# dusanerdeljan/stereo-depth

Measured on AMD Instinct MI355X. Metric: disparity maps/sec (stereo pairs/sec) at 1242x375 D=128, higher is better.
Workload: dtype f32

## Files before the change

stereo-depth_amd/build.py:

```python
from __future__ import annotations

import glob
import hashlib
import os
import shutil
import subprocess
import sys
from concurrent.futures import ThreadPoolExecutor

HERE = os.path.dirname(os.path.abspath(__file__))
CSRC = os.path.join(HERE, "csrc")
OBJ = os.path.join(CSRC, "build")
INCLUDE = os.path.join(os.path.dirname(HERE), "include")
LIB = os.path.join(HERE, "libstereo_mi355x.so")
FLAGS = ["--offload-arch=gfx950", "-O3", "-std=c++17", "-ffp-contract=off", "-fno-slp-vectorize", "-fPIC",
         "-Wall", "-Wno-pass-failed"]
PER_FILE_FLAGS = {"tu_capture.hip": ["-mllvm", "-pragma-unroll-threshold=65536"]}


def hipcc() -> str:
    for cand in (shutil.which("hipcc"), "/opt/rocm/bin/hipcc"):
        if cand and os.path.exists(cand):
            return cand
    raise RuntimeError("hipcc not found: cannot build libstereo_mi355x.so")


def sources():
    return sorted(glob.glob(os.path.join(CSRC, "*.hip")))


def _flags():
    extra = os.environ.get("SMX_EXTRA_FLAGS", "").split()
    return FLAGS + extra + ["-I", INCLUDE]


def _deps(depfile: str):
    try:
        txt = open(depfile).read().replace("\\\n", " ")
    except OSError:
        return None
    return [t for t in txt.split(":", 1)[1].split() if t]


def _stale(src: str, obj: str, stamp: str) -> bool:
    if not os.path.exists(obj):
        return True
    try:
        if open(obj + ".flags").read() != stamp:
            return True
    except OSError:
        return True
    deps = _deps(obj[:-2] + ".d")
    if deps is None:
        return True
    t = os.path.getmtime(obj)
    return any((not os.path.exists(d)) or os.path.getmtime(d) > t for d in deps + [src])


def build(force: bool = False, verbose: bool = False, variant: str = "") -> str:
    global LIB, OBJ
    if variant:
        LIB = os.path.join(HERE, f"libstereo_mi355x.{variant}.so")
        OBJ = os.path.join(CSRC, "build", variant)
    cc, flags = hipcc(), _flags()
    stamp = hashlib.sha256(" ".join([cc] + flags + [repr(sorted(PER_FILE_FLAGS.items()))]).encode()).hexdigest()
    try:
        fresh = (not force and open(LIB + ".flags").read() == stamp and
                 all(os.path.getmtime(f) <= os.path.getmtime(LIB)
                     for f in glob.glob(os.path.join(CSRC, "*.*")) + glob.glob(os.path.join(INCLUDE, "*.h")) + [__file__]))
    except OSError:
        fresh = False
    if fresh:
        return LIB
    os.makedirs(OBJ, exist_ok=True)
    jobs = []
    for src in sources():
        obj = os.path.join(OBJ, os.path.basename(src)[:-4] + ".o")
        if force or _stale(src, obj, stamp):
            jobs.append((src, obj))

    def compile_one(job):
        src, obj = job
        cmd = [cc] + flags + PER_FILE_FLAGS.get(os.path.basename(src), []) + ["-c", "-MD", "-MF", obj[:-2] + ".d", "-o", obj, src]
        if verbose:
            print(" ".join(cmd), flush=True)
        r = subprocess.run(cmd, capture_output=True, text=True)
        if r.returncode != 0:
            raise RuntimeError(f"hipcc failed on {os.path.basename(src)}:\n" + r.stdout + r.stderr)
        if r.stderr.strip() and verbose:
            print(r.stderr, file=sys.stderr)
        open(obj + ".flags", "w").write(stamp)

    if jobs:
        with ThreadPoolExecutor(max_workers=min(len(jobs), os.cpu_count() or 4, 8)) as pool:
            list(pool.map(compile_one, jobs))
    objs = [os.path.join(OBJ, os.path.basename(s)[:-4] + ".o") for s in sources()]
    if jobs or not os.path.exists(LIB) or any(os.path.getmtime(o) > os.path.getmtime(LIB) for o in objs):
        cmd = [cc, "--offload-arch=gfx950", "-shared", "-fPIC", "-o", LIB] + objs
        if verbose:
            print(" ".join(cmd), flush=True)
        r = subprocess.run(cmd, capture_output=True, text=True)
        if r.returncode != 0:
            raise RuntimeError("link failed:\n" + r.stdout + r.stderr)
    open(LIB + ".flags", "w").write(stamp)
    return LIB


if __name__ == "__main__":
    variant = next((a.split("=", 1)[1] for a in sys.argv if a.startswith("--variant=")), "")
    print(build(force="--force" in sys.argv, verbose="-v" in sys.argv or "--force" in sys.argv, variant=variant))
```

stereo-depth_amd/csrc/k_match_fast.h:

```cpp
#pragma once
#include "smx_common.h"

namespace smx {

constexpr int FA_HALO = 11;
constexpr int FA_VALID = 64 - 2 * FA_HALO;
#ifndef SMX_FA_WAVES
#define SMX_FA_WAVES 4
#endif
constexpr int FA_WAVES = SMX_FA_WAVES;
#ifndef SMX_FA_DS_WAVES
#define SMX_FA_DS_WAVES 8
#endif
constexpr int FA_DS_WAVES = SMX_FA_DS_WAVES;
#ifndef SMX_FA_TH
#define SMX_FA_TH 24
#endif
constexpr int FA_TH = SMX_FA_TH;
#ifndef SMX_FA_TH_SMALL
#define SMX_FA_TH_SMALL 8
#endif
constexpr int FA_TH_SMALL = SMX_FA_TH_SMALL;
constexpr int FA_TH_SMALL_TALL = 12;
constexpr int FA_TH_SMALL_MID = 10;
// ... 330 lines not shown
                            best[o] = __builtin_fmaxf(best[o], agg.x);
                            argb_update(o & 3, arg[o >> 2], agg.y, best[o], dvb);
                            best[o] = __builtin_fmaxf(best[o], agg.y);
                        } else {
                            const float m = __builtin_fmaxf(__builtin_fmaxf(best[o], agg.x), agg.y);
                            const int dsel = (agg.x == m) ? d : d + 1;
                            arg[o] = m > best[o] ? dsel : arg[o];
                            best[o] = m;
                        }
#endif
                    }
                }
            }
            s2 = s1;
            s1 = s0;
            k2 = k1;
            k1 = k0;
        }
        if ((rr_ % SMX_FA_SB_PERIOD) == SMX_FA_SB_PERIOD - 1)
            __builtin_amdgcn_sched_barrier(0);
    }
}

constexpr int FA_STAT_WG_STRIDE_DS = 16;
template <bool DSPLIT>
__device__ __forceinline__ void fast_stats_report(const MatchParams &p, int b, int wg_lin, int wv, int marches, bool window) {
    if (!p.fast_stats || b % p.fast_stride != 0) return;
    if (DSPLIT && wg_lin % FA_STAT_WG_STRIDE_DS != 0) return;
    const bool win = window && (!DSPLIT || wv == 0);
    const unsigned long long v = ((unsigned long long)(unsigned)marches << 24) | (win ? 1ull : 0ull);
    if (v != 0ull) (void)__hip_atomic_fetch_add(p.fast_stats, v, __ATOMIC_RELAXED, __HIP_MEMORY_SCOPE_AGENT);
}

template <int TH, int PR, bool P1ONLY, bool DSPLIT, int PK16, bool ARGB = false, bool DENSE = false>
__device__ __forceinline__ void match_fast_body(const MatchParams &p, const BlockIdx3 &blk) {
    static_assert(!DENSE || !P1ONLY, "the dense form is a pass 1 with neighbours: min_disparity = 0");
    static_assert(!DENSE || !DSPLIT || !ARGB, "latency shape: one register per winner");
    constexpr int NW = DSPLIT ? FA_DS_WAVES : FA_WAVES;
    constexpr int WGCOLS = DSPLIT ? 64 : FA_WGCOLS;
    constexpr int ND = PR - WGCOLS + 1;
    const int b = blk.z;

    extern __shared__ __attribute__((aligned(16))) unsigned short fsmem[];
    unsigned short *Lt = fsmem;
    unsigned short *Rt = fsmem + (TH + 22) * FA_PL;
    unsigned *bits = (unsigned *)(Rt + (TH + 22) * PR);
    const int BW = fast_bitwords(p.Dd);

    const int tid = threadIdx.x;
    const int lane = tid & 63;
    const int wv = tid >> 6;
    const int h = p.h, w = p.w, Dd = p.Dd;
    const int cwg0 = blk.x * (DSPLIT ? 1 : FA_WAVES) * FA_VALID;
    const int cw0 = cwg0 + (DSPLIT ? 0 : wv * FA_VALID);
    const int wcol = DSPLIT ? 0 : wv * FA_VALID;
    const bool active = cw0 < w;
    const int x0 = blk.y * TH;
    const int col = cw0 - FA_HALO + lane;
    const float *Lp = p.Ld + (size_t)b * h * w;
    const float *Rp = p.Rd + (size_t)b * h * w;
    const float unit = p.unit;

    FastLane ln;
    ln.xch = (float *)(bits + NW * BW) + wv * FA_XCH_FLOATS;
    ln.c255 = (unsigned)(255.0f * unit);
    ln.inv = 1.0f / (unit * unit * unit);
    ln.store_ok = active && lane >= FA_HALO && lane < FA_HALO + FA_VALID && col < w;
    ln.rows_ok = min(TH, h - x0);
    ln.plane = (size_t)p.B * h * w;
    ln.row0 = ((size_t)b * h + x0) * w;
    ln.colidx = ln.store_ok ? col : 0;
    ln.lptr = Lt + wcol + lane;

// ... 5 lines not shown
    float dfirst[DENSE && DSPLIT ? TH : 1];
#pragma unroll
    for (int o = 0; o < (DENSE ? TH : 1); ++o) { dmb[o] = 0.f; dma[o] = 0.f; dcp[o] = 0.f; }
#pragma unroll
    for (int o = 0; o < (DENSE && DSPLIT ? TH : 1); ++o) dfirst[o] = 0.f;

    fast_stage<(WGCOLS + 63) / 64, NW>(Lt, FA_PL, Lp, h, w, x0 - FA_HALO, cwg0 - FA_HALO, TH + 22, WGCOLS, unit, wv, lane);
    for (int e = tid; e < NW * BW; e += 64 * NW) bits[e] = 0u;

    auto stage_right = [&](int d0, int nd) {
        __syncthreads();
        const int cbase = cwg0 - FA_HALO - (p.dmin + d0 + nd - 1);
        fast_stage<(PR + 63) / 64, NW>(Rt, PR, Rp, h, w, x0 - FA_HALO, cbase, TH + 22, WGCOLS + nd - 1, unit, wv, lane);
        __syncthreads();
    };

    for (int d0 = 0; d0 < Dd; d0 += ND) {
        const int nd = min(ND, Dd - d0);
        stage_right(d0, nd);
        if (active) {
            const int q4 = ((nd + 2 * NW - 1) / (2 * NW)) * 2;
            const int dd_lo = DSPLIT ? min(nd, wv * q4) : 0;
            const int dd_hi = DSPLIT ? min(nd, dd_lo + q4) : nd;
            for (int dd = dd_lo; dd < dd_hi; dd += 2) {
                ln.rptr = Rt + wcol + lane + (nd - 1 - dd);
                if constexpr (DENSE)
                    fast_pass_pair<TH, PR, P1ONLY, PK16, 0, ARGB, true>(p, ln, d0 + dd, dd + 1 < dd_hi, best, arg, nullptr, 0, nullptr,
                                                                         0, 0, 0, 0, nullptr, nullptr, ~0u, dmb, dma, dcp,
                                                                         DSPLIT && dd == dd_lo ? dfirst : nullptr);
                else
                    fast_pass_pair<TH, PR, P1ONLY, PK16, 0, ARGB>(p, ln, d0 + dd, dd + 1 < dd_hi, best, arg);
            }
        }
    }
    if (ARGB) {
        int packed[(TH + 3) / 4];
#pragma unroll
        for (int o = 0; o < (TH + 3) / 4; ++o) packed[o] = arg[o];
#pragma unroll
        for (int o = 0; o < TH; ++o) arg[o] = (packed[o >> 2] >> (8 * (o & 3))) & 0xff;
    }
    float *mrg = (float *)(bits + NW * BW) + NW * FA_XCH_FLOATS;
    if constexpr (DSPLIT && DENSE) {
        constexpr int MR = fast_merge_rows(TH), R2 = (NW * MR * 2) / (NW * 6);
        static_assert(R2 >= 1 && R2 <= NW, "merge buffer: at least one row of six values per wave");
        const int q4 = ((Dd + 2 * NW - 1) / (2 * NW)) * 2;
        const int nk = (Dd + q4 - 1) / q4;
#pragma unroll 1
        for (int o0 = 0; o0 < TH; o0 += R2) {
            __syncthreads();
#pragma unroll
            for (int o = 0; o < TH; ++o) {
                if (o >= o0 && o < o0 + R2) {
                    float *q = mrg + ((size_t)(wv * R2 + (o - o0)) * 64 + lane) * 6;
                    q[0] = best[o]; q[1] = __int_as_float(arg[o]); q[2] = dmb[o]; q[3] = dma[o]; q[4] = dfirst[o]; q[5] = dcp[o];
                }
            }
            __syncthreads();
            const int j = wv;
            if (j < R2 && o0 + j < ln.rows_ok && ln.store_ok) {
                auto M = [&](int k, int f) { return mrg[((size_t)(k * R2 + j) * 64 + lane) * 6 + f]; };
                float bb = SMX_FLT_MIN;
                int aa = 0, kw = 0;
                for (int k = 0; k < nk; ++k) {
                    const float bk = M(k, 0);
                    const bool g = bk > bb;
// ... 174 lines not shown
#endif
    if (fl.form == FAST_DENSE_SMALL) {
        if constexpr (DSPLIT && TH == FA_TH_SMALL_TALL) launch_match_fast_k<TH, PR, false, true, false, true>(fl.pk, grid, block, lds, p, s);
    } else if (fl.form == FAST_DENSE) {
        if constexpr (!DSPLIT && ARGB && TH <= FA_DENSE_MAX_TH) launch_match_fast_k<TH, PR, false, false, ARGB, true>(fl.pk, grid, block, lds, p, s);
    } else if (fl.form == FAST_PASS1_ONLY) {
        launch_match_fast_k<TH, PR, true, DSPLIT, ARGB, false>(fl.pk, grid, block, lds, p, s);
    } else {
        launch_match_fast_k<TH, PR, false, DSPLIT, ARGB, false>(fl.pk, grid, block, lds, p, s);
    }
}

template <int TH, int PR, bool DSPLIT>
inline void launch_match_fast_t(const FastLaunch &fl, const MatchParams &p, int n, hipStream_t s) {
    if constexpr (DSPLIT) {
        launch_match_fast_a<TH, PR, true, false>(fl, p, n, s);
    } else if constexpr (PR == 256 || PR == FA_MID_PITCH) {
        launch_match_fast_a<TH, PR, false, true>(fl, p, n, s);
    } else {
        if (fl.argb) launch_match_fast_a<TH, PR, false, true>(fl, p, n, s);
        else launch_match_fast_a<TH, PR, false, false>(fl, p, n, s);
    }
}

__host__ __device__ constexpr int fast_tall_pitch(int Dd) { return Dd <= FA_WIDE_FROM ? 256 : (Dd <= FA_MID_UPTO ? FA_MID_PITCH : 320); }

template <int TH>
inline void launch_match_fast_tall(const FastLaunch &fl, const MatchParams &p, int n, hipStream_t s) {
    if (fl.pitch == 256) launch_match_fast_t<TH, 256, false>(fl, p, n, s);
    else if (fl.pitch == FA_MID_PITCH) launch_match_fast_t<TH, FA_MID_PITCH, false>(fl, p, n, s);
    else launch_match_fast_t<TH, 320, false>(fl, p, n, s);
}

struct FastPlan {
    bool small;
    int th;
    bool wide;
};

inline FastPlan match_fast_plan(const MatchParams &p, int n, int cus) {
    FastPlan pl{};
    const long wgs_tall = (long)((p.w + FA_VALID * FA_WAVES - 1) / (FA_VALID * FA_WAVES)) * ((p.h + FA_TH - 1) / FA_TH) * n;
    pl.small = 8 * wgs_tall < (p.on_lanes ? 8L : 13L) * cus;
    if (pl.small) {
        pl.th = FA_TH_SMALL;
        pl.wide = fast_small_wide(p.Dd);
        const long windows = (long)((p.w + FA_VALID - 1) / FA_VALID) * n;
        const long wg_small = windows * ((p.h + FA_TH_SMALL - 1) / FA_TH_SMALL), wg_tall = windows * ((p.h + FA_TH_SMALL_TALL - 1) / FA_TH_SMALL_TALL);
        if (wg_small > cus && wg_tall <= cus) {
            pl.th = FA_TH_SMALL_TALL;
#ifndef SMX_FA_NO_MID
#ifdef SMX_FA_MID_P1
        } else {
#else
        } else if (!p.pass1_only) {
#endif
            const long wg_mid = windows * ((p.h + FA_TH_SMALL_MID - 1) / FA_TH_SMALL_MID), slots = 2L * cus;
            const long r_small = (wg_small + slots - 1) / slots, r_mid = (wg_mid + slots - 1) / slots;
            if (r_mid * (FA_TH_SMALL_MID + 22) < r_small * (FA_TH_SMALL + 22)) pl.th = FA_TH_SMALL_MID;
#endif
        }
        return pl;
    }
    pl.wide = p.Dd > FA_WIDE_FROM;
    const int cand[3] = {24, 27, 32};
    int best = 24;
    long best_rows = -1;
    for (int th : cand) {
        const int pr = fast_tall_pitch(p.Dd);
        const size_t lds = pr == 256 ? fast_lds_bytes<256>(th, p.Dd) : (pr == FA_MID_PITCH ? fast_lds_bytes<FA_MID_PITCH>(th, p.Dd) : fast_lds_bytes<320>(th, p.Dd));
        const size_t granule = 1280;
        const bool three_per_cu = 3 * ((lds + granule - 1) / granule * granule) <= 160 * 1024;
        const long rows = (long)((p.h + th - 1) / th) * (th + 22) * (th == 32 ? 106 : 100) * (three_per_cu ? 100 : 130);
        if (best_rows < 0 || rows < best_rows) { best_rows = rows; best = th; }
    }
    pl.th = best;
#ifdef SMX_FA_FORCE_TH
    pl.th = SMX_FA_FORCE_TH;
#endif
    return pl;
}

}
```

stereo-depth_amd/csrc/smx_common.h:

```cpp
#pragma once

#include <hip/hip_runtime.h>
#include <stdint.h>

#define SMX_FLT_MIN 1.17549435e-38f

namespace smx {

__device__ __forceinline__ int wrapi(int g, int n) {
    g %= n;
    return g < 0 ? g + n : g;
}

__device__ __forceinline__ int pad_index_ref(int index, int n) {
    if (index >= 0 && index < n) return index;
    if (index < 0) return n + index;
    if (index == n) return 0;
    return n - index;
}

__device__ __forceinline__ float sum3_products(float a1, float b1, float a2, float b2, float a3, float b3, int conv) {
    float inner;
    if (conv == 1 || conv == 4) inner = __builtin_fmaf(a1, b1, a2 * b2);
    else if (conv == 2 || conv == 5) inner = __builtin_fmaf(a2, b2, a1 * b1);
// ... 131 lines not shown
    int nsplit;
    int pairs;
    float *slices;
    int pass1_only;
    int dense;
    int dense_small;
    unsigned long long *fast_stats;
    int fast_stride;
    int on_lanes;
    unsigned *tickets;
};

enum GateFlag { GATE_GRID_FLAG = 0, GATE_RANGE_FLAG };
enum ExactKernel { EXACT_GENERIC = 0, EXACT_GENERIC_VOLUME, EXACT_TILED };
struct ExactLaunch {
    int kernel = EXACT_GENERIC;
    int split = 1;
    int rows_per_thread = 4;
    int nd_chunk = 0;
    size_t lds_bytes = 0;
    size_t slice_floats = 0;
    int gate = 0, gate_flag = GATE_GRID_FLAG;
};
struct ExactCaptureLaunch { int split = 1, rows_per_thread = 4, nd_chunk = 0; size_t lds_bytes = 0; int gate = 0; };
enum FastForm { FAST_SPARSE = 0, FAST_PASS1_ONLY, FAST_DENSE, FAST_DENSE_SMALL, FAST_FORMS };
struct FastLaunch {
    int th = 0;
    bool small = false;
    int pitch = 0;
    int pk = 0;
    bool argb = false;
    int form = FAST_SPARSE;
    int gate = 0;
};
struct FastCaptureLaunch { bool small = false, wide = false; int pk = 0, gate = 0; };
struct AutoLaunch { int th = 0; bool wide = false; int pk = 0, nsplit = 1, nd_chunk = 0; size_t lds_bytes = 0; };
struct FilterLaunch { int th = 0; bool wide = false; int pk = 0; };
enum PrologueKernel { PROLOGUE_GENERIC = 0, PROLOGUE_K2, PROLOGUE_K4 };
struct PrologueLaunch { int in_mode = 0, kernel = PROLOGUE_GENERIC; };
enum RefineKind {
    REFINE_FLOAT = 0,
    REFINE_INT = 1,
    REFINE_INT_V = 2,
    REFINE_AUTO = 3,
    REFINE_AUTO_V = 4
};
struct RefineLaunch {
    int kind = REFINE_FLOAT;
    int kt = 0;
    bool apron = false;
    bool sad_exact = true;
};
enum FillKernel { FILL_4 = 0, FILL_POW2, FILL_GENERIC };
struct FillLaunch {
    int kernel = FILL_GENERIC, K = 1;
    int px = 8;
    int log2k = 0;
};

}
```

stereo-depth_amd/csrc/smx_engine.hip:

```cpp
#include <hip/hip_runtime.h>

#include <cstdarg>
#include <cstdio>
#include <cstdlib>
#include <cstring>
#include <mutex>
#include <new>
#include <string>
#include <vector>

#include "../../include/stereo_mi355x.h"
#include "k_fill.h"
#include "k_match_exact.h"
#include "k_match_exact2.h"
#include "k_match_auto.h"
#include "k_match_filter.h"
#include "k_match_capture.h"
#include "k_match_fast.h"
#include "k_prologue.h"
#include "k_refine.h"
#include "smx_common.h"
#include "smx_launch.h"
#include "smx_plan.h"
#include "smx_route.h"
// ... 105 lines not shown
        if (p) (void)hipFree(p);
    if (e->hints) (void)hipHostFree(e->hints);
    e->hints = e->hints_dev = nullptr;
}

struct SlotTimer {
    smx_engine *e;
    hipStream_t s;
    int lane, slot;
    bool on;
    SlotTimer(smx_engine *e_, hipStream_t s_, int lane_, int slot_) : e(e_), s(s_), lane(lane_), slot(slot_) {
        on = e->prof_on && e->prof_calls < e->prof_max;
        if (on) (void)hipEventRecord(e->prof_events[index() * 2], s);
    }
    size_t index() const { return ((size_t)e->prof_calls * smx_engine::LANES + lane) * SMX_KERNEL_SLOTS + slot; }
    ~SlotTimer() {
        if (on) {
            (void)hipEventRecord(e->prof_events[index() * 2 + 1], s);
            e->prof_used[index()] = 1;
        }
    }
};

using smx::SMX_EXACT2_LDS_CAP;
hipError_t raise_lds_caps(int device) {
    static std::mutex mu;
    static std::vector<int> done;
    std::lock_guard<std::mutex> lock(mu);
    for (int d : done)
        if (d == device) return hipSuccess;
    if (hipError_t e = smx::exact_raise_lds_caps(SMX_EXACT2_LDS_CAP + (int)((smx::E2_CAPBITS + 2 * smx::E2_SPARSE_WORDS) * sizeof(unsigned)));
        e != hipSuccess) return e;
    if (hipError_t e = smx::match_auto_raise_caps(); e != hipSuccess) return e;
    done.push_back(device);
    return hipSuccess;
}

bool env_is(const char *name, char c) {
    const char *v = std::getenv(name);
    return v && v[0] == c;
}

struct PairView {
    float *gray_l, *gray_r, *down_l, *down_r, *wta, *refined, *costs, *vol;
    int *flags, *flags2;
    uint8_t *gray8_l, *gray8_r;
    unsigned *cand;
};
PairView view_from(const smx_engine *e, int first) {
    const smx_dims &d = e->dm;
    const smx::EngineFacts &ef = e->facts;
    const size_t f = (size_t)first, hw = (size_t)d.h * d.w;
    PairView v{};
    v.gray_l = e->gray_l + f * d.H * ef.gpitch;
    v.gray_r = e->gray_r + f * d.H * ef.gpitch;
    v.down_l = e->down_l + f * hw;
    v.down_r = e->down_r + f * hw;
    v.wta = e->wta + f * hw;
    v.refined = e->refined + f * hw;
    v.costs = e->costs + f * hw;
    v.vol = e->vol ? e->vol + f * hw * d.Dd : nullptr;
    v.flags = e->flags + first;
    v.flags2 = e->flags + e->B + first;
    v.gray8_l = e->gray8_l ? e->gray8_l + f * d.H * ef.pitch8 : nullptr;
    v.gray8_r = e->gray8_r ? e->gray8_r + f * d.H * ef.pitch8 : nullptr;
    v.cand = e->cand ? e->cand + f * ef.cand_tiles_x * ef.cand_tiles_y * ef.cand_cw : nullptr;
// ... 477 lines not shown
    int ndev = 0;
    SMX_HIP(hipGetDeviceCount(&ndev));
    if (ndev <= 0)
        return fail(SMX_ERR_HIP, "no HIP device visible: libstereo_mi355x has no CPU fallback");
    if (cfg->device_id < 0 || cfg->device_id >= ndev)
        return fail(SMX_ERR_INVALID_CONFIG, "device_id %d outside [0, %d)", cfg->device_id, ndev);

    smx_engine *e = new (std::nothrow) smx_engine();
    if (!e) return fail(SMX_ERR_OUT_OF_MEMORY, "host allocation failed");
    e->cfg = *cfg;
    e->dm = d;
    e->B = cfg->max_batch > 0 ? cfg->max_batch : 1;
    {
        int nd = 0;
        const size_t need = smx::exact_tile_lds(*cfg, d.Dd, &nd);
        if (need > 64 * 1024) {
            delete e;
            return fail(SMX_ERR_UNSUPPORTED,
                        "radii too large for the LDS tile: ncc_patch_radius %u + large_mbm_radius %d need %zu bytes "
                        "of the 65536 available to the exact-order kernel",
                        cfg->ncc_patch_radius, cfg->large_mbm_radius, need);
        }
    }

    DeviceGuard guard(cfg->device_id);
    if (!guard.ok) {
        delete e;
        return fail(SMX_ERR_HIP, "cannot select HIP device %d", cfg->device_id);
    }
    int cus = 0;
    if (hipDeviceGetAttribute(&cus, hipDeviceAttributeMultiprocessorCount, cfg->device_id) != hipSuccess || cus <= 0) cus = 256;
    smx::PlanOptions opt;
    opt.fast_dense = env_is("SMX_FAST_DENSE", '1') ? 1 : (env_is("SMX_FAST_DENSE", '0') ? 0 : -1);
    opt.fast_dense_small = env_is("SMX_FAST_DENSE_SMALL", '1') ? 1 : (env_is("SMX_FAST_DENSE_SMALL", '0') ? 0 : -1);
    e->opt_lane_priority = env_is("SMX_LANE_PRIORITY", '0') ? 0 : 1;
    e->opt_debug_hints = std::getenv("SMX_DEBUG_HINTS") != nullptr;
    if (const char *v = std::getenv("SMX_TEST_EPOCH_START")) {
        const long k = std::atol(v);
        if (k > 0 && k < 0x7fffffffL) e->epoch = (int)k;
    }
    e->facts = smx::derive_facts(*cfg, d, cus, opt);
    const smx::EngineFacts &f = e->facts;
    e->overlap_min = cfg->overlap_min_pairs < 0 ? 0
                     : (cfg->overlap_min_pairs > 0 ? (cfg->overlap_min_pairs < 2 ? 2 : cfg->overlap_min_pairs) : overlap_min_pairs_default(f));
    const size_t B = (size_t)e->B, hw = (size_t)d.h * d.w;
    hipError_t err = hipSuccess;
    auto alloc = [&](void **p, size_t bytes) {
        if (err == hipSuccess) err = hipMalloc(p, bytes);
        if (err == hipSuccess) err = hipMemset(*p, 0, bytes);
    };
    alloc((void **)&e->gray_l, B * (size_t)d.H * f.gpitch * sizeof(float));
    alloc((void **)&e->gray_r, B * (size_t)d.H * f.gpitch * sizeof(float));
    alloc((void **)&e->down_l, B * hw * sizeof(float));
    alloc((void **)&e->down_r, B * hw * sizeof(float));
    alloc((void **)&e->wta, B * hw * sizeof(float));
    alloc((void **)&e->refined, B * hw * sizeof(float));
    alloc((void **)&e->costs, 3 * B * hw * sizeof(float));
    alloc((void **)&e->flags, 2 * B * sizeof(int));
    alloc((void **)&e->fast_stats_dev, smx_engine::LANES * sizeof(unsigned long long));
    if (f.has_u8_planes()) {
        alloc((void **)&e->gray8_l, B * (size_t)d.H * f.pitch8);
        alloc((void **)&e->gray8_r, B * (size_t)d.H * f.pitch8);
    }
    if (f.has_tickets()) alloc((void **)&e->tickets, B * (size_t)f.e2_tiles * sizeof(unsigned));
    if (f.has_slices()) {
        alloc((void **)&e->slices, smx_engine::LANES * f.slices_floats * sizeof(float));
// ... 246 lines not shown
```

stereo-depth_amd/csrc/smx_launch.h:

```cpp
#pragma once
#include <hip/hip_runtime.h>
#include <stdint.h>

#include "smx_common.h"

namespace smx {

struct RefineParams;
struct FillParams;
struct FilterParams;

struct PrologueArgs {
    const void *left, *right;
    float *gray_l, *gray_r, *down_l, *down_r;
    int *flags, *flags2;
    uint8_t *g8_l, *g8_r;
    int H, W, K, h, w, grid_capable, pitch8, padl, padr, epoch, gpitch, gpadl;
    int fp_conv;
};
void launch_prologue(const PrologueLaunch &x, const PrologueArgs &a, int n, hipStream_t s);
void launch_refine(const RefineLaunch &x, const RefineParams &p, int n, hipStream_t s);
void launch_fill(const FillLaunch &x, const FillParams &p, int n, hipStream_t s);
void launch_flag_to_bool(const int *flag, int epoch, int *out, hipStream_t s);
void launch_metrics(int n, const float *est, const float *gt, const uint8_t *mask, size_t pixels, float max_disparity,
                    const float thresholds[4], double *out_sums, hipStream_t s);
void launch_points(const float *disp, int H, int W, float bf, float invalid, float *depth, float *points, int *count_dev,
                   int *workspace, hipStream_t s);

void launch_exact(const ExactLaunch &x, const MatchParams &p, int n, hipStream_t s);
void launch_exact2_capture(const ExactCaptureLaunch &x, const MatchParams &p, int n, hipStream_t s);
void launch_exact2_sparse(const MatchParams &p, int n, unsigned *cand, int cw, const int *range_flags, unsigned *stats_dev,
                          unsigned long long *stats_host, unsigned seq, hipStream_t s);
hipError_t exact_raise_lds_caps(int cap_bytes);

void launch_match_fast(const FastLaunch &fl, const MatchParams &p, int n, hipStream_t s);
void launch_match_fast_tall_24(const FastLaunch &fl, const MatchParams &p, int n, hipStream_t s);
void launch_match_fast_tall_27(const FastLaunch &fl, const MatchParams &p, int n, hipStream_t s);
void launch_match_fast_tall_32(const FastLaunch &fl, const MatchParams &p, int n, hipStream_t s);
void launch_match_auto_small_tu(const AutoLaunch &al, const MatchParams &p, int n, hipStream_t s);
hipError_t match_auto_raise_caps();

void launch_match_capture_tu(const FastCaptureLaunch &cl, const MatchParams &p, int n, hipStream_t s);

void launch_match_filter_tu(const FilterLaunch &fl, const MatchParams &p, const FilterParams &f, int n, hipStream_t s);
void launch_match_filter_24(const FilterLaunch &fl, const MatchParams &p, const FilterParams &f, int n, hipStream_t s);
void launch_match_filter_27(const FilterLaunch &fl, const MatchParams &p, const FilterParams &f, int n, hipStream_t s);
void launch_match_filter_32(const FilterLaunch &fl, const MatchParams &p, const FilterParams &f, int n, hipStream_t s);

void launch_lr_pack(int elem_bytes, const void *l, const void *r, void *pl, void *pr, long rows, int W, hipStream_t s);
void launch_lr_check(bool mirrored, const float *left, const float *right, float *out, float *right_out, int n, int H, int W,
                     float max_diff, float invalid, hipStream_t s);

void launch_filter_speckles(int n, int H, int W, const float *in, float *out, int max_size, float max_diff, float invalid,
                            void *workspace, hipStream_t s);
void launch_fill_invalid(int n, int H, int W, const float *in, float *out, float invalid, void *workspace, hipStream_t s);

size_t median_workspace_bytes(int n, int H, int W);
void launch_weighted_median(int n, int H, int W, const float *in, const float *holes, const float *guide, float *out,
                            int radius, const uint16_t *range, const uint16_t *spatial, float invalid, hipStream_t s);

void launch_wls(int n, int H, int W, const float *in, const float *conf, const float *guide, float *out, int iterations,
                const float *lambdas, const float *range, float min_weight, float invalid, void *workspace,
                hipStream_t s);

void launch_confidence(int n, int H, int W, const float *left, const float *right, const float *guide, int radius,
                       float lr_scale, float texture_scale, float invalid, float *out, hipStream_t s);

void launch_temporal(int n, int H, int W, const float *disp, const float *conf, const float *guide,
                     const float *prev_guide, float *state_disp, float *state_weight, float *guide_out, float *out,
                     int radius, float threshold, float decay, float max_diff, float max_weight, float min_weight,
                     float invalid, hipStream_t s);
// ... 49 lines not shown
```

stereo-depth_amd/csrc/smx_plan.h:

```cpp
#pragma once

#include "../../include/stereo_mi355x.h"
#include "k_match_auto.h"
#include "k_match_capture.h"
#include "k_match_exact.h"
#include "k_match_exact2.h"
#include "k_match_fast.h"
#include "k_match_filter.h"
#include "k_prologue.h"
#include "smx_common.h"
#include "smx_launch.h"
#include "smx_route.h"

namespace smx {

constexpr int SMX_EXACT2_LDS_CAP = 80 * 1024;

struct PlanOptions {
    int fast_dense = -1;
    int fast_dense_small = -1;
};

struct EngineFacts {
    int match_mode = SMX_MATCH_AUTO, exact_filter = 0;
    int B = 1, h = 0, w = 0, dmin = 0, Dd = 0, K = 1;
    int sad_patch_radius = 5;
    int cus = 256;
    PlanOptions opt;
    bool grid_capable = false;
    bool default_radii = false;
    bool fast_ok = false;
    bool filter_ok = false;
    bool capture = false;
    bool has_volume = false;
    int kt = 0;
    int pitch8 = 0, padl = 0, padr = 0;
    int gpitch = 0, gpadl = 0;
    bool prologue_k2 = false;
    bool prologue_k4 = false;
    bool sad_exact = true;
    int exact_nd = 0, exact2_nd = 0;
    size_t exact_lds = 0, exact2_lds = 0;
    int e2_tiles = 0;
    size_t slices_floats = 0;
    int cand_tiles_x = 0, cand_tiles_y = 0, cand_cw = 0;
    int filter_unit = 0;
    float filter_two_e = 0.f;
    bool filter_words = false, fast_words = false;

    bool has_u8_planes() const { return pitch8 != 0; }
    bool has_tickets() const { return default_radii; }
    bool has_slices() const { return slices_floats != 0; }
};
// ... 86 lines not shown
    AggRoute route = AGG_EXACT;
    bool gated_dense_first = false;
    bool exact_split = false;
    bool capture_follows = false;
    FastPlan fast{};
    bool dense = false, dense_small = false;
    bool reports = false;
    int stride = 0;
    bool fill_publishes = false;
    bool owns_gray = true;
    bool refine_reports_grid = false;
    PrologueLaunch prologue{};
    RefineLaunch refine{};
    FillLaunch fill{};
    ExactLaunch exact{};
    ExactCaptureLaunch exact_capture{};
    FastLaunch fast_launch{};
    FastCaptureLaunch fast_capture{};
    AutoLaunch auto_launch{};
    FilterLaunch filter{};

    bool has_fast_launch() const { return route == AGG_FAST || route == AGG_AUTO_ONE_LAUNCH || route == AGG_AUTO_GATED; }
};

inline bool is_rgb(int in_mode) { return in_mode == IN_RGB_F32 || in_mode == IN_RGB_U8; }

inline MatchParams plan_params(const EngineFacts &f, bool on_lanes) {
    MatchParams mp{};
    mp.B = f.B; mp.h = f.h; mp.w = f.w; mp.dmin = f.dmin; mp.Dd = f.Dd;
    mp.on_lanes = on_lanes ? 1 : 0;
    mp.pass1_only = f.capture ? 1 : 0;
    return mp;
}
inline FastPlan range_fast_plan(const EngineFacts &f, bool on_lanes, int n) { return match_fast_plan(plan_params(f, on_lanes), n, f.cus); }

inline ExactLaunch exact_launch(const EngineFacts &f, bool on_lanes, int n, bool allow_split) {
    ExactLaunch x;
    if (!f.default_radii || f.has_volume) {
        x.kernel = f.has_volume ? EXACT_GENERIC_VOLUME : EXACT_GENERIC;
        x.nd_chunk = f.exact_nd;
        x.lds_bytes = f.exact_lds;
        return x;
    }
    x.kernel = EXACT_TILED;
    x.nd_chunk = f.exact2_nd;
    x.lds_bytes = f.exact2_lds;
    x.split = allow_split ? exact_split(f.e2_tiles, n, f.Dd, f.cus) : 1;
    if (x.split > 1) {
        x.slice_floats = (size_t)x.split * SMX_SLICE_WORDS * n * f.h * f.w;
        const int per = (f.Dd + x.split - 1) / x.split;
        if (x.nd_chunk > per) x.nd_chunk = per;
        const long wgs = (long)f.e2_tiles * n * x.split, slots = 2L * f.cus;
        x.rows_per_thread = on_lanes && 2 * wgs > slots && wgs < 2 * slots ? 4 : 2;
    }
    return x;
}

inline ExactCaptureLaunch exact_capture_launch(const EngineFacts &f, int n, bool allow_split) {
    ExactCaptureLaunch x;
    x.split = allow_split ? capture_split(f.e2_tiles, n, f.Dd, f.cus) : 1;
    x.rows_per_thread = allow_split ? 2 : 4;
    x.nd_chunk = f.exact2_nd;
    x.lds_bytes = exact2_capture_lds_bytes(f.exact2_nd);
    return x;
}

inline FastLaunch fast_launch(const EngineFacts &f, const FastPlan &pl, bool dense, bool dense_small) {
    FastLaunch x;
    x.small = pl.small;
    x.th = pl.th;
    x.pk = fast_pk(f.K * f.K);
    bool dense_here;
    if (pl.small) {
        x.pitch = pl.wide ? 320 : 256;
        dense_here = dense_small && pl.th == FA_TH_SMALL_TALL && f.Dd <= x.pitch - 64 + 1;
    } else {
        x.pitch = fast_tall_pitch(f.Dd);
        x.argb = x.pitch != 320 || f.Dd <= 256;
        if (pl.th == 32 && dense && !f.capture && f.Dd <= 256) x.th = FA_DENSE_MAX_TH;
        dense_here = dense && x.argb && x.th <= FA_DENSE_MAX_TH;
    }
    x.form = f.capture ? FAST_PASS1_ONLY : (!dense_here ? FAST_SPARSE : (pl.small ? FAST_DENSE_SMALL : FAST_DENSE));
    return x;
}

inline FastCaptureLaunch fast_capture_launch(const EngineFacts &f, const FastPlan &pl) {
    return FastCaptureLaunch{pl.small, f.Dd > FA_WIDE_FROM, fast_pk(f.K * f.K)};
}

inline AutoLaunch auto_launch(const EngineFacts &f, const MatchParams &mp, int th) {
    AutoLaunch x;
    x.th = th;
    x.wide = fast_small_wide(f.Dd);
    x.pk = fast_pk(f.K * f.K);
    x.nsplit = match_auto_nsplit(mp, th);
    x.nd_chunk = f.exact2_nd;
    const int per = (f.Dd + x.nsplit - 1) / x.nsplit;
    if (x.nd_chunk > per) x.nd_chunk = per;
    x.lds_bytes = x.wide ? fast_lds_bytes<320>(th, f.Dd, true) : fast_lds_bytes<256>(th, f.Dd, true);
    const size_t exact_lds = exact2_lds_floats(x.nd_chunk) * sizeof(float);
    if (exact_lds > x.lds_bytes) x.lds_bytes = exact_lds;
    return x;
}

inline FilterLaunch filter_launch(const EngineFacts &f, const MatchParams &mp, int n) {
    const FilterPlan pl = filter_plan(mp, n, f.cus);
    return FilterLaunch{pl.th, pl.wide, fast_pk(f.filter_unit)};
}

inline PrologueLaunch prologue_launch(const EngineFacts &f, const CallFacts &call) {
    const bool u8 = call.in_mode == IN_GRAY_U8 || call.in_mode == IN_RGB_U8;
    PrologueLaunch x;
    x.in_mode = call.in_mode;
    if (f.prologue_k2 && !is_rgb(call.in_mode)) x.kernel = PROLOGUE_K2;
    else if (f.prologue_k4 && (!u8 || call.u8_aligned)) x.kernel = PROLOGUE_K4;
// ... 4 lines not shown
    FillLaunch x;
    x.K = f.K;
    x.kernel = f.K == 1 || f.K == 2 || f.K == 4 ? FILL_4 : ((f.K & (f.K - 1)) == 0 ? FILL_POW2 : FILL_GENERIC);
    x.px = on_lanes && n > 4 ? 4 : 8;
    while ((1 << x.log2k) < f.K) x.log2k++;
    return x;
}

inline RangePlan plan_range(const EngineFacts &f, const CallFacts &call, int n, bool whole_call) {
    RangePlan p;
    p.owns_gray = call.in_mode != IN_GRAY_F32;
    p.prologue = prologue_launch(f, call);
    if (f.match_mode == SMX_MATCH_FAST_GRID && !f.fast_ok) {
        p.status = SMX_ERR_UNSUPPORTED;
        p.refusal = "SMX_MATCH_FAST_GRID needs downscale_factor in {1,2,4,8}, ncc radius 1 and "
                    "block-matching radii 1/4/10";
        return p;
    }
    if (f.has_volume && f.match_mode == SMX_MATCH_FAST_GRID) {
        p.status = SMX_ERR_UNSUPPORTED;
        p.refusal = "SMX_MATCH_FAST_GRID cannot serve min_disparity/K > disparity count or "
                    "non-default radii with min_disparity > 0 (aggregated volume needed)";
        return p;
    }
    const bool rgb = is_rgb(call.in_mode);
    p.mode = f.match_mode;
    if (f.has_volume) p.mode = SMX_MATCH_EXACT_ORDER;
    if (p.mode == SMX_MATCH_AUTO) {
        if (!f.fast_ok) p.mode = SMX_MATCH_EXACT_ORDER;
        else if (call.in_mode == IN_GRAY_U8) p.mode = SMX_MATCH_FAST_GRID;
        else if (rgb) p.mode = SMX_MATCH_EXACT_ORDER;
    }
    const MatchParams mp = plan_params(f, call.on_lanes);
    p.fast = match_fast_plan(mp, n, f.cus);
    const bool small = p.fast.small;
    p.capture_follows = f.capture;

    if (p.mode == SMX_MATCH_EXACT_ORDER && f.filter_ok && rgb && !small && f.default_radii && call.route.use_filter) {
        p.route = AGG_FILTERED;
        p.gated_dense_first = call.in_mode == IN_RGB_F32;
        p.filter = filter_launch(f, mp, n);
    } else if (p.mode == SMX_MATCH_EXACT_ORDER) {
        p.route = AGG_EXACT;
        p.exact_split = whole_call;
    } else if (p.mode == SMX_MATCH_FAST_GRID) {
        p.route = AGG_FAST;
    } else {
        const bool one_launch = f.default_radii && small && call.route.grid_hint == 0 && !f.capture && !f.has_volume && f.has_tickets() &&
                                f.has_slices() && match_auto_small_applicable(mp, p.fast.th, n, f.slices_floats);
        if (one_launch) {
            p.route = AGG_AUTO_ONE_LAUNCH;
            p.auto_launch = auto_launch(f, mp, p.fast.th);
        } else {
            p.route = AGG_AUTO_GATED;
            p.exact_split = whole_call && small && call.route.grid_hint != 0;
        }
    }

    if (p.has_fast_launch() && !mp.pass1_only && f.Dd <= FA_BITWORDS * 32) {
        const bool tall12 = small && p.fast.th == FA_TH_SMALL_TALL;
        if (!small || tall12) {
            if (!(tall12 && f.opt.fast_dense_small == 1) && f.fast_words && f.opt.fast_dense < 0) {
                p.stride = n > 4 ? (n + 3) / 4 : 1;
                const long wgs_pair = tall12 ? (long)((f.w + FA_VALID - 1) / FA_VALID) * ((f.h + p.fast.th - 1) / p.fast.th)
                                             : (long)((f.w + FA_VALID * FA_WAVES - 1) / (FA_VALID * FA_WAVES)) * ((f.h + 23) / 24) * FA_WAVES;
                p.reports = ((n + p.stride - 1) / p.stride) * wgs_pair < (1L << 23);
            }
            const bool dense = tall12 && f.opt.fast_dense_small >= 0 ? f.opt.fast_dense_small == 1 : call.route.fast_dense;
            if (dense) (tall12 ? p.dense_small : p.dense) = true;
            else p.fill_publishes = p.reports;
        }
    }

    if (p.route == AGG_FILTERED || p.route == AGG_EXACT || p.route == AGG_AUTO_GATED) {
        p.exact = exact_launch(f, call.on_lanes, n, p.exact_split);
        if (p.capture_follows) p.exact_capture = exact_capture_launch(f, n, p.exact_split);
    }
    if (p.route == AGG_FAST || p.route == AGG_AUTO_GATED) {
        p.fast_launch = fast_launch(f, p.fast, p.dense, p.dense_small);
        if (p.capture_follows) p.fast_capture = fast_capture_launch(f, p.fast);
    }
    if (p.route == AGG_FILTERED) {
        p.exact.gate = 2;
        p.exact.gate_flag = GATE_RANGE_FLAG;
    } else if (p.route == AGG_AUTO_GATED) {
        p.exact.gate = p.exact_capture.gate = 2;
        p.fast_launch.gate = p.fast_capture.gate = 1;
    }

    p.refine.kt = f.kt;
    p.refine.sad_exact = f.sad_exact;
    if (f.kt == 0 || !f.has_u8_planes() || rgb) {
        p.refine.kind = REFINE_FLOAT;
        p.refine.apron = p.owns_gray && f.gpadl > 0 && call.in_mode != IN_GRAY_U8;
    } else if (call.in_mode == IN_GRAY_U8) {
        p.refine.kind = n > 4 ? REFINE_INT_V : REFINE_INT;
    } else if (n <= 4) {
        p.refine.kind = REFINE_AUTO;
        p.refine_reports_grid = whole_call;
    } else {
        p.refine.kind = REFINE_AUTO_V;
    }
    p.fill = fill_launch(f, call.on_lanes, n);
    return p;
}
// ... 43 lines not shown
inline MatchParams filter_params(const RangeParams &b, const EngineFacts &f) {
    MatchParams p = b.mp;
    p.unit = (float)f.filter_unit;
    return p;
}
inline MatchParams sparse_params(const RangeParams &b, const EngineFacts &f) {
    MatchParams p = b.mp;
    p.nd_chunk = f.exact2_nd;
    return p;
}

inline CallKind call_kind(const EngineFacts &f, int in_mode, bool on_lanes, int n0, int n1) {
    CallKind k{};
    CallFacts call;
    call.in_mode = in_mode;
    call.on_lanes = on_lanes;
    for (int n : {n0, n1}) {
        if (n < 1) continue;
        const RangePlan p = plan_range(f, call, n, n1 < 1);
        if (p.status != SMX_OK) continue;
        if (p.route == AGG_FILTERED && f.filter_words) k.filter_reports = true;
        if (p.has_fast_launch() && p.reports) k.fast_reports = true;
    }
    return k;
}

inline void match_geometry(const EngineFacts &f, bool on_lanes, int n, smx_match_geometry *g) {
    if (!f.fast_ok) {
        g->kernel = SMX_KERNEL_EXACT_ONLY;
        return;
    }
    const FastPlan pl = range_fast_plan(f, on_lanes, n);
    g->kernel = pl.small ? SMX_KERNEL_FAST_SPLIT : SMX_KERNEL_FAST_WINDOW;
    g->band_rows = pl.th;
    g->waves_per_workgroup = pl.small ? FA_DS_WAVES : FA_WAVES;
    const int cols_per_wg = FA_VALID * (pl.small ? 1 : FA_WAVES);
    const long wgs = (long)((f.w + cols_per_wg - 1) / cols_per_wg) * ((f.h + pl.th - 1) / pl.th);
    g->rows_marched = g->band_rows + 22;
    g->workgroups = (int)(wgs * n);
    const long waves = wgs * g->waves_per_workgroup;
    const double lane_rows = (double)waves * 64.0 * g->rows_marched / (g->kernel == SMX_KERNEL_FAST_SPLIT ? (double)FA_DS_WAVES : 1.0);
    g->useful_fraction = (double)f.h * f.w / lane_rows;
    g->columns_per_wave = (double)f.w * ((f.h + g->band_rows - 1) / g->band_rows) /
                          ((double)waves / (g->kernel == SMX_KERNEL_FAST_SPLIT ? (double)FA_DS_WAVES : 1.0));
}

}
```

stereo-depth_amd/csrc/tu_fast_small.hip:

```cpp
#include "k_match_auto.h"
#include "k_match_filter.h"
#include "smx_launch.h"

namespace smx {

void launch_match_fast(const FastLaunch &fl, const MatchParams &p, int n, hipStream_t s) {
    if (fl.small) {
        if (fl.th == FA_TH_SMALL_TALL) {
            if (fl.pitch == 256) launch_match_fast_t<FA_TH_SMALL_TALL, 256, true>(fl, p, n, s);
            else launch_match_fast_t<FA_TH_SMALL_TALL, 320, true>(fl, p, n, s);
        } else if (fl.th == FA_TH_SMALL_MID) {
            if (fl.pitch == 256) launch_match_fast_t<FA_TH_SMALL_MID, 256, true>(fl, p, n, s);
            else launch_match_fast_t<FA_TH_SMALL_MID, 320, true>(fl, p, n, s);
        } else {
            if (fl.pitch == 256) launch_match_fast_t<FA_TH_SMALL, 256, true>(fl, p, n, s);
            else launch_match_fast_t<FA_TH_SMALL, 320, true>(fl, p, n, s);
        }
    } else if (fl.th == 27) {
        launch_match_fast_tall_27(fl, p, n, s);
    } else if (fl.th == 32) {
        launch_match_fast_tall_32(fl, p, n, s);
    } else {
        launch_match_fast_tall_24(fl, p, n, s);
    }
}

void launch_match_auto_small_tu(const AutoLaunch &al, const MatchParams &p, int n, hipStream_t s) { launch_match_auto_small(al, p, n, s); }

hipError_t match_auto_raise_caps() { return match_auto_raise_lds_caps(MATCH_AUTO_LDS_CAP); }

void launch_match_filter_tu(const FilterLaunch &fl, const MatchParams &p, const FilterParams &f, int n, hipStream_t s) {
    switch (fl.th) {
        case 24: launch_match_filter_24(fl, p, f, n, s); break;
        case 32: launch_match_filter_32(fl, p, f, n, s); break;
        default: launch_match_filter_27(fl, p, f, n, s); break;
    }
}

}
```

Measured before the change: 92430.

## Add stacked double-height fast-match bands to amortize halo rows

Adds a fast-match kernel variant that processes two 24-row unit bands per workgroup (48 rows). This amortizes the 22 halo rows marched per band and reduces workgroup count. Pass 2 runs per unit band from byte-packed winners, and the variant is compiled in its own unit with a VGPR cap and a build check that rejects scratch spills. The planner picks it on lanes when the total marched rows drop, at the cost of higher register and LDS pressure and lower occupancy.

New measurement: 99500, median of 6. 1.08x the previous value.

```diff
diff --git a/stereo-depth_amd/build.py b/stereo-depth_amd/build.py
--- a/stereo-depth_amd/build.py
+++ b/stereo-depth_amd/build.py
@@ -3,6 +3,7 @@
 import glob
 import hashlib
 import os
+import re
 import shutil
 import subprocess
 import sys
@@ -15,7 +16,9 @@
 LIB = os.path.join(HERE, "libstereo_mi355x.so")
 FLAGS = ["--offload-arch=gfx950", "-O3", "-std=c++17", "-ffp-contract=off", "-fno-slp-vectorize", "-fPIC",
          "-Wall", "-Wno-pass-failed"]
-PER_FILE_FLAGS = {"tu_capture.hip": ["-mllvm", "-pragma-unroll-threshold=65536"]}
+PER_FILE_FLAGS = {"tu_capture.hip": ["-mllvm", "-pragma-unroll-threshold=65536"],
+                  "tu_fast_stack.hip": ["-mllvm", "-pragma-unroll-threshold=65536", "-Rpass-analysis=kernel-resource-usage"]}
+NO_SCRATCH = {"tu_fast_stack.hip"}
 
 
 def hipcc() -> str:
@@ -27,6 +30,21 @@
 
 def sources():
     return sorted(glob.glob(os.path.join(CSRC, "*.hip")))
+
+
+def check_resources(unit: str, remarks: str) -> None:
+    name, seen = None, 0
+    for line in remarks.splitlines():
+        m = re.search(r"remark:\s+(Function Name|ScratchSize \[bytes/lane\]|SGPRs Spill|VGPRs Spill): (\S+)", line)
+        if not m:
+            continue
+        if m.group(1) == "Function Name":
+            name = m.group(2)
+            seen += "k_match_fast" in name
+        elif name and "k_match_fast" in name and int(m.group(2)) != 0:
+            raise RuntimeError(f"{unit}: {name} reports {m.group(1)} = {m.group(2)}: the march must stay in registers")
+    if seen == 0:
+        raise RuntimeError(f"{unit}: no resource remarks for k_match_fast (is -Rpass-analysis=kernel-resource-usage still among its flags?)")
 
 
 def _flags():
@@ -89,6 +107,8 @@
             raise RuntimeError(f"hipcc failed on {os.path.basename(src)}:\n" + r.stdout + r.stderr)
         if r.stderr.strip() and verbose:
             print(r.stderr, file=sys.stderr)
+        if os.path.basename(src) in NO_SCRATCH:
+            check_resources(os.path.basename(src), r.stderr)
         open(obj + ".flags", "w").write(stamp)
 
     if jobs:
diff --git a/stereo-depth_amd/csrc/k_match_fast.h b/stereo-depth_amd/csrc/k_match_fast.h
--- a/stereo-depth_amd/csrc/k_match_fast.h
+++ b/stereo-depth_amd/csrc/k_match_fast.h
@@ -386,6 +386,93 @@
     if (v != 0ull) (void)__hip_atomic_fetch_add(p.fast_stats, v, __ATOMIC_RELAXED, __HIP_MEMORY_SCOPE_AGENT);
 }
 
+template <int TU, int NH, int PR, int PK16, class StageRight>
+__device__ __forceinline__ void fast_stacked_tail(const MatchParams &p, const BlockIdx3 &blk, const FastLane &ln, const float (&best)[TU * NH],
+                                                  const int (&argb)[TU * NH], const unsigned short *Rt, unsigned *bits, int wcol, int x0,
+                                                  bool active, StageRight &&stage_right) {
+    constexpr int ND = PR - FA_WGCOLS + 1;
+    const int lane = threadIdx.x & 63, wv = threadIdx.x >> 6;
+    const int h = p.h, w = p.w, Dd = p.Dd, BW = fast_bitwords(Dd);
+    const bool all_needed = Dd > FA_BITWORDS * 32;
+    unsigned *wbits = bits + wv * BW;
+#pragma unroll
+    for (int hh = 0; hh < NH; ++hh) {
+        float bh[TU];
+        int ah[TU];
+#pragma unroll
+        for (int o = 0; o < TU; ++o) {
+            bh[o] = best[hh * TU + o];
+            ah[o] = (argb[(hh * TU + o) >> 2] >> (8 * ((hh * TU + o) & 3))) & 0xff;
+        }
+        FastLane lh = ln;
+        lh.lptr = ln.lptr + hh * TU * FA_PL;
+        lh.row0 = ln.row0 + (size_t)(hh * TU) * w;
+        lh.rows_ok = max(0, min(TU, h - x0 - hh * TU));
+        const unsigned short *Rh = Rt + hh * TU * PR;
+        unsigned dup_left = 0u;
+#ifndef SMX_FA_NO_DEDUP
+        if (!all_needed) {
+#pragma unroll
+            for (int o = 0; o < TU; ++o) {
+                const int la = __builtin_amdgcn_update_dpp(-1, ah[o], 0x138, 0xf, 0xf, false);
+                dup_left |= (la == ah[o] ? 1u : 0u) << o;
+            }
+            const int left_ok = __builtin_amdgcn_update_dpp(0, lh.store_ok ? 1 : 0, 0x138, 0xf, 0xf, false);
+            if (!left_ok) dup_left = 0u;
+        }
+#endif
+        if (lh.store_ok) {
+#pragma unroll
+            for (int o = 0; o < TU; ++o) {
+                if (o < lh.rows_ok) {
+                    const unsigned off = (unsigned)(o * w + lh.colidx);
+                    store_u32off(p.wta + lh.row0, off, (float)ah[o] + (float)p.dmin);
+                    const bool nv = !(bh[o] > SMX_FLT_MIN);
+                    store_u32off(p.costs + lh.row0, off, nv ? 0.0f : bh[o] * lh.inv);
+                    if (!all_needed && !((dup_left >> o) & 1u)) {
+                        const int dn = (ah[o] + 1 == Dd) ? 0 : ah[o] + 1;
+                        const int dp = (ah[o] == 0) ? Dd - 1 : ah[o] - 1;
+                        atomicOr(&wbits[dn], 1u << o);
+                        atomicOr(&wbits[dp], 1u << o);
+                    }
+                }
+            }
+        }
+        int marches2 = 0;
+        unsigned argpk[(TU + 1) / 2];
+#pragma unroll
+        for (int o = 0; o < (TU + 1) / 2; ++o) argpk[o] = 0u;
+#pragma unroll
+        for (int o = 0; o < TU; ++o)
+            argpk[o >> 1] |= ((lh.store_ok && o < lh.rows_ok) ? (unsigned)ah[o] : 0xffffu) << (16 * (o & 1));
+        for (int d0 = 0; d0 < Dd; d0 += ND) {
+            const int nd = min(ND, Dd - d0);
+            if (Dd > ND) stage_right(d0, nd);
+            else __syncthreads();
+            if (active) {
+                auto march = [&](int dda, int ddb, unsigned rows) {
+                    const int da = d0 + dda, db = d0 + ddb;
+                    ++marches2;
+                    lh.rptr = Rh + wcol + lane + (nd - 1 - dda);
+                    fast_pass_pair<TU, PR, false, PK16, 1>(p, lh, da, false, bh, ah, Rh + wcol + lane + (nd - 1 - ddb), db, argpk,
+                                                           da == 0 ? Dd - 1 : da - 1, da + 1 == Dd ? 0 : da + 1,
+                                                           db == 0 ? Dd - 1 : db - 1, db + 1 == Dd ? 0 : db + 1, nullptr, nullptr, rows);
+                };
+                int pend = -1;
+                unsigned pend_rows = 0u;
+                SMX_FOR_EACH_NEEDED(wbits + d0, 0, nd, all_needed, lane, dd, rows, {
+                    if (pend < 0) { pend = dd; pend_rows = rows; }
+                    else { march(pend, dd, pend_rows | rows); pend = -1; }
+                })
+                if (pend >= 0) march(pend, pend, pend_rows);
+            }
+        }
+        if (lane == 0) fast_stats_report<false>(p, blk.z, (int)(blk.x + gridDim.x * blk.y), wv, marches2, active && lh.rows_ok > 0);
+        if (hh + 1 < NH)
+            for (int e = lane; e < BW; e += 64) wbits[e] = 0u;
+    }
+}
+
 template <int TH, int PR, bool P1ONLY, bool DSPLIT, int PK16, bool ARGB = false, bool DENSE = false>
 __device__ __forceinline__ void match_fast_body(const MatchParams &p, const BlockIdx3 &blk) {
     static_assert(!DENSE || !P1ONLY, "the dense form is a pass 1 with neighbours: min_disparity = 0");
@@ -393,6 +480,10 @@
     constexpr int NW = DSPLIT ? FA_DS_WAVES : FA_WAVES;
     constexpr int WGCOLS = DSPLIT ? 64 : FA_WGCOLS;
     constexpr int ND = PR - WGCOLS + 1;
+    constexpr int NH = TH > 32 ? 2 : 1;
+    constexpr int TU = TH / NH;
+    static_assert(NH == 1 || (TH == 2 * TU && TU <= 32 && ARGB && !DSPLIT && !DENSE && !P1ONLY),
+                  "stacked bands: two unit bands, byte-packed winners, throughput shape, sparse form");
     const int b = blk.z;
 
     extern __shared__ __attribute__((aligned(16))) unsigned short fsmem[];
@@ -464,6 +555,10 @@
                     fast_pass_pair<TH, PR, P1ONLY, PK16, 0, ARGB>(p, ln, d0 + dd, dd + 1 < dd_hi, best, arg);
             }
         }
+    }
+    if constexpr (NH > 1) {
+        fast_stacked_tail<TU, NH, PR, PK16>(p, blk, ln, best, arg, Rt, bits, wcol, x0, active, stage_right);
+        return;
     }
     if (ARGB) {
         int packed[(TH + 3) / 4];
@@ -704,13 +799,42 @@
     else launch_match_fast_t<TH, 320, false>(fl, p, n, s);
 }
 
+constexpr int FA_STACK = 2;
+constexpr int FA_STACK_TH = FA_STACK * FA_TH;
+template <int PR> inline bool fast_stack_fits(int Dd) {
+    const size_t granule = 1280, lds = fast_lds_bytes<PR>(FA_STACK_TH, Dd);
+    return 2 * ((lds + granule - 1) / granule * granule) <= 160 * 1024;
+}
+inline bool fast_stack_instantiated(int pitch, int Dd) { return pitch == 256 && fast_stack_fits<256>(Dd); }
+
+template <int PR>
+inline void launch_match_fast_stacked(const FastLaunch &fl, const MatchParams &p, int n, hipStream_t s) {
+    const dim3 grid((p.w + FA_VALID * FA_WAVES - 1) / (FA_VALID * FA_WAVES), (p.h + FA_STACK_TH - 1) / FA_STACK_TH, n);
+    const size_t lds = fast_lds_bytes<PR>(FA_STACK_TH, p.Dd);
+    const dim3 block(64 * FA_WAVES);
+    if (fl.pk == 2) hipLaunchKernelGGL((k_match_fast<FA_STACK_TH, PR, false, false, 2, true, false>), grid, block, lds, s, p);
+    else if (fl.pk == 1) hipLaunchKernelGGL((k_match_fast<FA_STACK_TH, PR, false, false, 1, true, false>), grid, block, lds, s, p);
+    else hipLaunchKernelGGL((k_match_fast<FA_STACK_TH, PR, false, false, 0, true, false>), grid, block, lds, s, p);
+}
+template <int PR>
+inline hipError_t fast_stacked_raise_lds_caps() {
+    const int cap = (int)fast_lds_bytes<PR>(FA_STACK_TH, PR - FA_WGCOLS + 1);
+    const void *kernels[3] = {reinterpret_cast<const void *>(&k_match_fast<FA_STACK_TH, PR, false, false, 2, true, false>),
+                              reinterpret_cast<const void *>(&k_match_fast<FA_STACK_TH, PR, false, false, 1, true, false>),
+                              reinterpret_cast<const void *>(&k_match_fast<FA_STACK_TH, PR, false, false, 0, true, false>)};
+    for (const void *k : kernels)
+        if (hipError_t e = hipFuncSetAttribute(k, hipFuncAttributeMaxDynamicSharedMemorySize, cap); e != hipSuccess) return e;
+    return hipSuccess;
+}
+
 struct FastPlan {
     bool small;
     int th;
     bool wide;
+    int stack = 1;
 };
 
-inline FastPlan match_fast_plan(const MatchParams &p, int n, int cus) {
+inline FastPlan match_fast_plan(const MatchParams &p, int n, int cus, int stack_opt = -1) {
     FastPlan pl{};
     const long wgs_tall = (long)((p.w + FA_VALID * FA_WAVES - 1) / (FA_VALID * FA_WAVES)) * ((p.h + FA_TH - 1) / FA_TH) * n;
     pl.small = 8 * wgs_tall < (p.on_lanes ? 8L : 13L) * cus;
@@ -750,6 +874,13 @@
 #ifdef SMX_FA_FORCE_TH
     pl.th = SMX_FA_FORCE_TH;
 #endif
+    if (stack_opt != 0 && !p.dense && !p.pass1_only && fast_stack_instantiated(fast_tall_pitch(p.Dd), p.Dd)) {
+        const long rows_stack = (long)((p.h + FA_STACK_TH - 1) / FA_STACK_TH) * (FA_STACK_TH + 22);
+        if (stack_opt == 1 || (p.on_lanes && rows_stack < (long)((p.h + pl.th - 1) / pl.th) * (pl.th + 22))) {
+            pl.th = FA_TH;
+            pl.stack = FA_STACK;
+        }
+    }
     return pl;
 }
 
diff --git a/stereo-depth_amd/csrc/smx_common.h b/stereo-depth_amd/csrc/smx_common.h
--- a/stereo-depth_amd/csrc/smx_common.h
+++ b/stereo-depth_amd/csrc/smx_common.h
@@ -187,6 +187,7 @@
     bool argb = false;
     int form = FAST_SPARSE;
     int gate = 0;
+    int stack = 1;
 };
 struct FastCaptureLaunch { bool small = false, wide = false; int pk = 0, gate = 0; };
 struct AutoLaunch { int th = 0; bool wide = false; int pk = 0, nsplit = 1, nd_chunk = 0; size_t lds_bytes = 0; };
diff --git a/stereo-depth_amd/csrc/smx_engine.hip b/stereo-depth_amd/csrc/smx_engine.hip
--- a/stereo-depth_amd/csrc/smx_engine.hip
+++ b/stereo-depth_amd/csrc/smx_engine.hip
@@ -161,6 +161,7 @@
     if (hipError_t e = smx::exact_raise_lds_caps(SMX_EXACT2_LDS_CAP + (int)((smx::E2_CAPBITS + 2 * smx::E2_SPARSE_WORDS) * sizeof(unsigned)));
         e != hipSuccess) return e;
     if (hipError_t e = smx::match_auto_raise_caps(); e != hipSuccess) return e;
+    if (hipError_t e = smx::fast_stack_raise_caps(); e != hipSuccess) return e;
     done.push_back(device);
     return hipSuccess;
 }
@@ -704,6 +705,7 @@
     if (hipDeviceGetAttribute(&cus, hipDeviceAttributeMultiprocessorCount, cfg->device_id) != hipSuccess || cus <= 0) cus = 256;
     smx::PlanOptions opt;
     opt.fast_dense = env_is("SMX_FAST_DENSE", '1') ? 1 : (env_is("SMX_FAST_DENSE", '0') ? 0 : -1);
+    opt.fast_stack = env_is("SMX_FAST_STACK", '1') ? 1 : (env_is("SMX_FAST_STACK", '0') ? 0 : -1);
     opt.fast_dense_small = env_is("SMX_FAST_DENSE_SMALL", '1') ? 1 : (env_is("SMX_FAST_DENSE_SMALL", '0') ? 0 : -1);
     e->opt_lane_priority = env_is("SMX_LANE_PRIORITY", '0') ? 0 : 1;
     e->opt_debug_hints = std::getenv("SMX_DEBUG_HINTS") != nullptr;
diff --git a/stereo-depth_amd/csrc/smx_launch.h b/stereo-depth_amd/csrc/smx_launch.h
--- a/stereo-depth_amd/csrc/smx_launch.h
+++ b/stereo-depth_amd/csrc/smx_launch.h
@@ -37,6 +37,8 @@
 void launch_match_fast_tall_24(const FastLaunch &fl, const MatchParams &p, int n, hipStream_t s);
 void launch_match_fast_tall_27(const FastLaunch &fl, const MatchParams &p, int n, hipStream_t s);
 void launch_match_fast_tall_32(const FastLaunch &fl, const MatchParams &p, int n, hipStream_t s);
+void launch_match_fast_stack(const FastLaunch &fl, const MatchParams &p, int n, hipStream_t s);
+hipError_t fast_stack_raise_caps();
 void launch_match_auto_small_tu(const AutoLaunch &al, const MatchParams &p, int n, hipStream_t s);
 hipError_t match_auto_raise_caps();
 
diff --git a/stereo-depth_amd/csrc/smx_plan.h b/stereo-depth_amd/csrc/smx_plan.h
--- a/stereo-depth_amd/csrc/smx_plan.h
+++ b/stereo-depth_amd/csrc/smx_plan.h
@@ -19,6 +19,7 @@
 struct PlanOptions {
     int fast_dense = -1;
     int fast_dense_small = -1;
+    int fast_stack = -1;
 };
 
 struct EngineFacts {
@@ -171,7 +172,7 @@
     mp.pass1_only = f.capture ? 1 : 0;
     return mp;
 }
-inline FastPlan range_fast_plan(const EngineFacts &f, bool on_lanes, int n) { return match_fast_plan(plan_params(f, on_lanes), n, f.cus); }
+inline FastPlan range_fast_plan(const EngineFacts &f, bool on_lanes, int n) { return match_fast_plan(plan_params(f, on_lanes), n, f.cus, f.opt.fast_stack); }
 
 inline ExactLaunch exact_launch(const EngineFacts &f, bool on_lanes, int n, bool allow_split) {
     ExactLaunch x;
@@ -220,6 +221,7 @@
         dense_here = dense && x.argb && x.th <= FA_DENSE_MAX_TH;
     }
     x.form = f.capture ? FAST_PASS1_ONLY : (!dense_here ? FAST_SPARSE : (pl.small ? FAST_DENSE_SMALL : FAST_DENSE));
+    x.stack = pl.stack;
     return x;
 }
 
@@ -290,7 +292,7 @@
         else if (rgb) p.mode = SMX_MATCH_EXACT_ORDER;
     }
     const MatchParams mp = plan_params(f, call.on_lanes);
-    p.fast = match_fast_plan(mp, n, f.cus);
+    p.fast = match_fast_plan(mp, n, f.cus, f.opt.fast_stack);
     const bool small = p.fast.small;
     p.capture_follows = f.capture;
 
@@ -329,6 +331,11 @@
             else p.fill_publishes = p.reports;
         }
     }
+    if (p.dense && p.fast.stack > 1) {
+        MatchParams md = mp;
+        md.dense = 1;
+        p.fast = match_fast_plan(md, n, f.cus, f.opt.fast_stack);
+    }
 
     if (p.route == AGG_FILTERED || p.route == AGG_EXACT || p.route == AGG_AUTO_GATED) {
         p.exact = exact_launch(f, call.on_lanes, n, p.exact_split);
@@ -438,10 +445,10 @@
     }
     const FastPlan pl = range_fast_plan(f, on_lanes, n);
     g->kernel = pl.small ? SMX_KERNEL_FAST_SPLIT : SMX_KERNEL_FAST_WINDOW;
-    g->band_rows = pl.th;
+    g->band_rows = pl.th * pl.stack;
     g->waves_per_workgroup = pl.small ? FA_DS_WAVES : FA_WAVES;
     const int cols_per_wg = FA_VALID * (pl.small ? 1 : FA_WAVES);
-    const long wgs = (long)((f.w + cols_per_wg - 1) / cols_per_wg) * ((f.h + pl.th - 1) / pl.th);
+    const long wgs = (long)((f.w + cols_per_wg - 1) / cols_per_wg) * ((f.h + g->band_rows - 1) / g->band_rows);
     g->rows_marched = g->band_rows + 22;
     g->workgroups = (int)(wgs * n);
     const long waves = wgs * g->waves_per_workgroup;
diff --git a/stereo-depth_amd/csrc/tu_fast_small.hip b/stereo-depth_amd/csrc/tu_fast_small.hip
--- a/stereo-depth_amd/csrc/tu_fast_small.hip
+++ b/stereo-depth_amd/csrc/tu_fast_small.hip
@@ -16,6 +16,8 @@
             if (fl.pitch == 256) launch_match_fast_t<FA_TH_SMALL, 256, true>(fl, p, n, s);
             else launch_match_fast_t<FA_TH_SMALL, 320, true>(fl, p, n, s);
         }
+    } else if (fl.stack == FA_STACK) {
+        launch_match_fast_stack(fl, p, n, s);
     } else if (fl.th == 27) {
         launch_match_fast_tall_27(fl, p, n, s);
     } else if (fl.th == 32) {
diff --git a/stereo-depth_amd/csrc/tu_fast_stack.hip b/stereo-depth_amd/csrc/tu_fast_stack.hip
--- /dev/null
+++ b/stereo-depth_amd/csrc/tu_fast_stack.hip
@@ -0,0 +1,14 @@
+#define SMX_FA_OCC 2
+#define SMX_FA_NUM_VGPR 192
+#include "k_match_fast.h"
+#include "smx_launch.h"
+
+namespace smx {
+constexpr int REFINE_AUTO_V2_VGPRS = 120;
+static_assert(2 * SMX_FA_NUM_VGPR + REFINE_AUTO_V2_VGPRS <= 512, "two stacked aggregation waves and one step-6 wave share a SIMD");
+
+void launch_match_fast_stack(const FastLaunch &fl, const MatchParams &p, int n, hipStream_t s) {
+    launch_match_fast_stacked<256>(fl, p, n, s);
+}
+hipError_t fast_stack_raise_caps() { return fast_stacked_raise_lds_caps<256>(); }
+}
```
